# cbg-ethz/metMHN

Measured on AMD Instinct MI355X. Metric: full-cohort log-lik+grad evals/sec at n=20 events; kronvec HBM GB/s, higher is better.
Workload: dtype f64

## Files before the change

### include/metmhn_amd.h

```cpp
#ifndef METMHN_AMD_H
#define METMHN_AMD_H

#include <stddef.h>
#include <stdint.h>

#ifdef __cplusplus
extern "C" {
#endif

typedef struct mmhn_engine* mmhn_handle;

enum { MMHN_F64 = 0, MMHN_F32 = 1 };

int mmhn_create(int device_id, int n_mut, int dtype, mmhn_handle* out);
void mmhn_destroy(mmhn_handle h);
const char* mmhn_last_error(void);
int mmhn_set_workspace_limit(mmhn_handle h, size_t bytes);

int mmhn_set_cohort(mmhn_handle h, const int8_t* dat, int64_t n_pat, int n_cols);
int mmhn_score(mmhn_handle h, const double* log_theta, const double* log_d_p, const double* log_d_m,
               double perc_met, double* score);
int mmhn_score_and_grad(mmhn_handle h, const double* log_theta, const double* log_d_p,
                        const double* log_d_m, double perc_met, double* score, double* d_theta,
                        double* d_dp, double* d_dm);
// ... 83 lines not shown
                         double* pos_mt, int32_t* status);

int mmhn_order_samples(mmhn_handle h, const double* log_theta, const double* obs1, const double* obs2, const int8_t* dat,
                       int64_t n_pat, int n_cols, int64_t first, int64_t n_samples, uint64_t seed, double* log_evidence,
                       int8_t* orders, double* log_prob, int32_t* status);

enum { MMHN_K_OTHER_SOLVE = 0,
       MMHN_K_PSOLVE_FWD = 1,
       MMHN_K_PSOLVE_ADJ = 2,
       MMHN_K_PCLASS = 3,
       MMHN_K_CSOLVE_FWD = 4,
       MMHN_K_CSOLVE_ADJ = 5,
       MMHN_K_COUNT = 6 };
typedef struct {
  double ms;
  int64_t launches;
  double alg_bytes;
} mmhn_kernel_counter;
typedef struct {
  mmhn_kernel_counter kernel[MMHN_K_COUNT];
  double eval_ms;
  int64_t evals;
  int32_t comm_ranks;
  int32_t comm_rank;
} mmhn_counters;
#define MMHN_ABI_VERSION 8
int mmhn_abi_version(void);
int mmhn_bench_kronvec(mmhn_handle h, const double* log_theta, const int8_t* state, int64_t batch,
                       int iters, int transpose, int jacobi, double* ms_per_launch, int64_t* tiles);
int mmhn_bench_stream(mmhn_handle h, size_t bytes, int iters, int kind, double* gbps);
int mmhn_get_counters(mmhn_handle h, mmhn_counters* out);
int mmhn_reset_counters(mmhn_handle h);
int mmhn_debug_lane_moves(mmhn_handle h, int transposed, int* out);

#ifdef __cplusplus
}
#endif
#endif
```

### metmhn_amd/_lib.py

```python
from __future__ import annotations

import ctypes as C
import os
import subprocess

_HERE = os.path.dirname(os.path.abspath(__file__))
_ROOT = os.path.dirname(_HERE)
import glob
_SRC = [os.path.join(_HERE, "csrc", "engine.hip")] + sorted(glob.glob(os.path.join(_HERE, "csrc", "*.h")))
_HDR = os.path.join(_ROOT, "include", "metmhn_amd.h")
LIB_PATH = os.environ.get("MMHN_LIB", os.path.join(_HERE, "libmetmhn_amd.so"))

f64p = C.POINTER(C.c_double)
i8p = C.POINTER(C.c_int8)
i64p = C.POINTER(C.c_int64)
i32p = C.POINTER(C.c_int32)


KERNEL_CLASSES = ("other_solve", "psolve_fwd", "psolve_adj", "pclass", "csolve_fwd", "csolve_adj")


class KernelCounter(C.Structure):
    _fields_ = [("ms", C.c_double), ("launches", C.c_int64), ("alg_bytes", C.c_double)]

# ... 14 lines not shown
    "mmhn_cohort_sums_end": [C.c_void_p, f64p],
    "mmhn_cohort_wsums_begin": [C.c_void_p, f64p, f64p, f64p, C.c_int, C.c_double],
    "mmhn_cohort_wsums_end": [C.c_void_p, f64p],
    "mmhn_set_reduce_flag": [C.c_void_p, C.c_double],
    "mmhn_get_reduce_flag": [C.c_void_p, f64p],
    "mmhn_patient_grads": [C.c_void_p, f64p, f64p, f64p, f64p, f64p, f64p, f64p],
    "mmhn_kronvec": [C.c_void_p, f64p, i8p, f64p, f64p, C.c_int, C.c_int],
    "mmhn_kronvec_batched": [C.c_void_p, f64p, i8p, C.c_int64, f64p, f64p, C.c_int, C.c_int],
    "mmhn_jacobi_step_batched": [C.c_void_p, f64p, f64p, f64p, i8p, C.c_int64, f64p, f64p, f64p, C.c_int],
    "mmhn_kron_diag": [C.c_void_p, f64p, i8p, f64p],
    "mmhn_diag_scal": [C.c_void_p, f64p, i8p, f64p, f64p, C.c_int],
    "mmhn_obs_states": [C.c_void_p, i8p, C.c_int, i64p, i64p],
    "mmhn_resolvent": [C.c_void_p, f64p, f64p, f64p, i8p, f64p, f64p, C.c_int],
    "mmhn_x_partial_Q_y": [C.c_void_p, f64p, i8p, f64p, f64p, f64p],
    "mmhn_x_partial_D_y": [C.c_void_p, f64p, f64p, i8p, f64p, f64p, f64p, f64p],
    "mmhn_partial_diag_scal": [C.c_void_p, f64p, i8p, f64p, C.c_int, C.c_int, f64p],
    "mmhn_v_kronvec": [C.c_void_p, f64p, i8p, f64p, f64p, C.c_int, C.c_int],
    "mmhn_v_resolvent": [C.c_void_p, f64p, i8p, f64p, f64p, f64p, C.c_int],
    "mmhn_v_x_partial_Q_y": [C.c_void_p, f64p, i8p, f64p, f64p, f64p, f64p],
    "mmhn_v_kron_diag": [C.c_void_p, f64p, i8p, f64p, f64p],
    "mmhn_v_scal_d_pt": [C.c_void_p, f64p, f64p, i8p, f64p, f64p, f64p],
    "mmhn_v_d_scal_d_pt": [C.c_void_p, f64p, f64p, i8p, f64p, C.c_int, f64p, f64p],
    "mmhn_v_x_partial_D_y": [C.c_void_p, f64p, f64p, i8p, f64p, f64p, f64p, f64p],
    "mmhn_comm_unique_id": [C.c_void_p],
    "mmhn_comm_init": [C.c_void_p, C.c_void_p, C.c_int, C.c_int],
    "mmhn_comm_destroy": [C.c_void_p],
    "mmhn_bench_stream": [C.c_void_p, C.c_size_t, C.c_int, C.c_int, f64p],
    "mmhn_bench_kronvec": [C.c_void_p, f64p, i8p, C.c_int64, C.c_int, C.c_int, C.c_int, f64p, i64p],
    "mmhn_simulate": [C.c_void_p, f64p, f64p, f64p, C.c_int64, C.c_uint64, i8p, i8p],
    "mmhn_simulate_summary": [C.c_void_p, f64p, f64p, f64p, C.c_int64, C.c_int64, C.c_uint64, i64p],
    "mmhn_get_counters": [C.c_void_p, C.POINTER(Counters)],
    "mmhn_reset_counters": [C.c_void_p],
    "mmhn_debug_lane_moves": [C.c_void_p, C.c_int, C.POINTER(C.c_int)],
    "mmhn_likeliest_orders": [C.c_void_p, f64p, f64p, f64p, i8p, C.c_int64, C.c_int, C.c_int, i8p, f64p, i32p],
    "mmhn_order_posteriors": [C.c_void_p, f64p, f64p, f64p, i8p, C.c_int64, C.c_int, f64p, f64p, f64p, i32p],
    "mmhn_order_precedences": [C.c_void_p, f64p, f64p, f64p, i8p, C.c_int64, C.c_int, f64p, f64p, i32p],
    "mmhn_order_positions": [C.c_void_p, f64p, f64p, f64p, i8p, C.c_int64, C.c_int, f64p, f64p, f64p, i32p],
    "mmhn_order_samples": [C.c_void_p, f64p, f64p, f64p, i8p, C.c_int64, C.c_int, C.c_int64, C.c_int64, C.c_uint64, f64p, i8p,
                           f64p, i32p],
}
OTHER_SYMBOLS = ("mmhn_destroy", "mmhn_last_error", "mmhn_abi_version")
ABI_VERSION = 8


def needs_build() -> bool:
    if not os.path.exists(LIB_PATH):
        return True
    t = os.path.getmtime(LIB_PATH)
    return any(os.path.exists(s) and os.path.getmtime(s) > t for s in _SRC + [_HDR])


def build(force: bool = False, verbose: bool = False) -> str:
    if not force and not needs_build():
        return LIB_PATH
    hipcc = os.environ.get("HIPCC", "/opt/rocm/bin/hipcc")
    cmd = [hipcc, "-O3", "-std=c++17", "--offload-arch=gfx950", "-shared", "-fPIC", "-Wno-comment",
           "-o", LIB_PATH, _SRC[0]]
    if verbose:
        print(" ".join(cmd))
    res = subprocess.run(cmd, capture_output=True, text=True)
    if res.returncode != 0:
        raise RuntimeError("hipcc failed:\n" + res.stderr)
    return LIB_PATH


_lib = None
# ... 39 lines not shown
```

### metmhn_amd/csrc/engine.hip

```cpp
#include <algorithm>
#include <chrono>
#include <cmath>
#include <cstdio>
#include <cstdlib>
#include <cstring>
#include <string>
#include <vector>

#include "../../include/metmhn_amd.h"
#include "host.h"
#include "comm.h"
#include "plan.h"
#include "sampler.h"

namespace mmhn {

static thread_local std::string g_err;

struct CListDev {
  DevArr<CItem> items;
  DevArr<int> deps;
};
struct StagedDev {
  DevArr<int> pats, paired, probs;
// ... 87 lines not shown
  DevArr<T> piM, qM;
  DevArr<T> zarena;
  struct View { T* p = nullptr; } GJ, DJ, Abuf;
  int pi_owner = -1, qJ_owner = -1;
  DevArr<double> lp, out, sums, abi_sums, redbuf;
  DevArr<JLink<T>> links;
  double* h_abi = nullptr;
  double* h_abi_dev = nullptr;
  hipStream_t side[3] = {};
  hipEvent_t ev_fork[3] = {}, ev_join[3] = {};
  bool small_forked[2] = {false, false}, fork_recorded[2] = {false, false};
  DevArr<CoopCtl> coop_ctl;
  DevArr<unsigned> coop_flags[2];
  unsigned coop_epoch = 0;
  int coop_slot = 0;
  int cur_lane = 0;
  unsigned* h_abort = nullptr;
  unsigned* h_abort_dev = nullptr;
  bool coop_used = false;
  bool coop_alone = false;
  bool sums_pending = false;
  std::chrono::steady_clock::time_point sums_t0, sums_issued;
  int sums_len = 0;
  int pack_mode = 0;
  double pack_a = 0, pack_b = 0;
  double* pack_dst = nullptr;
  bool packed_in_eval = false;
  double reduce_flag = 0.0, reduce_flag_sum = 0.0;
  bool flag_pending = false;
  ncclComm_t comm = nullptr;
  int comm_rank = 0, comm_size = 1;
  bool time_kernels = true;
  mmhn_counters cnt{};
  std::vector<std::pair<hipEvent_t, hipEvent_t>> ev_pool;
  size_t ev_used = 0;
  std::vector<double> ev_bytes;
  std::vector<int> ev_slot;

  static long long zarena_elems(long long nJ, long long asize, int N) { return up4(3 * nJ * N * N) + up4(3 * nJ * N) + up4(asize); }
  static long long zclear_elems(const Batch& b, int N) { return zarena_elems((long long)b.dJ.size(), b.aclr, N); }

  Engine(int dev_id, int n_mut) : n(n_mut), N(n_mut + 1) {
    device = dev_id;
    cnt.comm_rank = -1;
    REQUIRE(n_mut >= 1 && n_mut < MAXN, "n_mut must be in [1, 31]");
    DevGuard guard(device);
    HIPCHECK(hipStreamCreateWithFlags(&stream, hipStreamNonBlocking));
    d_par.alloc(NPSET);
    HIPCHECK(hipHostMalloc(reinterpret_cast<void**>(&h_par), NPSET * sizeof(Params<T>), hipHostMallocDefault));
    HIPCHECK(hipHostGetDevicePointer(&h_par_dev, h_par, 0));
    static_assert(sizeof(Params<T>) % sizeof(uint4) == 0, "parameter block: whole 16-byte words");
    sums.alloc(2 * stride());
    size_t free_b = 0, total_b = 0;
    HIPCHECK(hipMemGetInfo(&free_b, &total_b));
    cfg.plan.ws_limit = (size_t)(0.7 * (double)free_b);
    hipDeviceProp_t prop;
    HIPCHECK(hipGetDeviceProperties(&prop, device));
    cfg.plan.n_cu = std::max(1, prop.multiProcessorCount);
    {
      std::vector<uint16_t> perm((size_t)(TB + 1) << TB, 0);
      std::vector<int> lvl((size_t)(TB + 1) * (TB + 2), 0);
      for (int t = 0; t <= TB; ++t) {
        int pos = 0;
        for (int l = 0; l <= t; ++l) {
          lvl[(size_t)t * (TB + 2) + l] = pos;
          for (uint32_t x = 0; x < (1u << t); ++x)
            if (popc(x) == l) perm[((size_t)t << TB) + pos++] = (uint16_t)x;
        }
        lvl[(size_t)t * (TB + 2) + t + 1] = pos;
      }
      d_perm.alloc(perm.size());
      d_lvl.alloc(lvl.size());
      HIPCHECK(hipMemcpy(d_perm.p, perm.data(), perm.size() * sizeof(uint16_t), hipMemcpyHostToDevice));
      HIPCHECK(hipMemcpy(d_lvl.p, lvl.data(), lvl.size() * sizeof(int), hipMemcpyHostToDevice));
    }
    raise_lds(wsolve_lds<T>(), &k_wsolve<T, false>, &k_wsolve<T, true>, &k_wsolve<T, false, WCfg<T>::NXT>, &k_wsolve<T, true, WCfg<T>::NXT>);
    raise_lds(wclass_lds<T>(), &k_wclass<T>);
    raise_lds(160 * 1024, &k_spatient2<T>, &k_spatient<T, 1024, 1>);
    raise_lds(150 * 1024,
              &k_csolve<T, false, false>, &k_csolve<T, true, false>, &k_csolve<T, false, true>, &k_csolve<T, true, true>,
              &k_csolve<T, false, false, 4>, &k_csolve<T, true, false, 4>,
              &k_psolve2<T, false, true>, &k_psolve2<T, true, true>, &k_psolve2<T, false, false>, &k_psolve2<T, true, false>,
              &k_tsolve<T, false, false>, &k_tsolve<T, true, false>, &k_tsolve<T, false, true>, &k_tsolve<T, true, true>,
              &k_kv<T, false, 1, false>, &k_kv<T, true, 1, false>, &k_kv<T, false, 1, true>, &k_kv<T, true, 1, true>,
              &k_sweep<T, false>, &k_sweep<T, true>, &k_diag<T>, &k_diag<T, 1024>,
              &k_prep<T, false>, &k_prep<T, true>, &k_prep<T, false, 1024>, &k_grad_rows<T, 1>, &k_grad_rows<T>,
              &k_pclass<T, false>, &k_pclass<T, true>, &k_class_marg<T>);
    coop_ctl.alloc(1);
    HIPCHECK(hipMemset(coop_ctl.p, 0, sizeof(CoopCtl)));
    HIPCHECK(hipHostMalloc(reinterpret_cast<void**>(&h_abort), 64, hipHostMallocDefault));
    HIPCHECK(hipHostGetDevicePointer(reinterpret_cast<void**>(&h_abort_dev), h_abort, 0));
    *h_abort = 0u;
    for (int i = 0; i < 3; ++i) {
      HIPCHECK(hipStreamCreateWithFlags(&side[i], hipStreamNonBlocking));
      HIPCHECK(hipEventCreateWithFlags(&ev_fork[i], hipEventDisableTiming));
      HIPCHECK(hipEventCreateWithFlags(&ev_join[i], hipEventDisableTiming));
    }
  }
  ~Engine() override {
    comm_destroy();
    for (auto& e : ev_pool) { (void)hipEventDestroy(e.first); (void)hipEventDestroy(e.second); }
    for (int i = 0; i < 3; ++i) {
      if (ev_join[i]) (void)hipEventDestroy(ev_join[i]);
      if (ev_fork[i]) (void)hipEventDestroy(ev_fork[i]);
      if (side[i]) (void)hipStreamDestroy(side[i]);
    }
    if (h_par) (void)hipHostFree(h_par);
    if (h_abi) (void)hipHostFree(h_abi);
    if (h_abort) (void)hipHostFree(h_abort);
    if (stream) (void)hipStreamDestroy(stream);
    stream = nullptr;
  }
  int stride() const { return 1 + N * N + 2 * N; }

  void build_params(const double* lt, const double* ldp, const double* ldm, bool upload = true) {
    REQUIRE(!sums_pending, "an evaluation begun with mmhn_cohort_sums_begin has not been collected (its parameter upload may still be in flight)");
    std::vector<double> eth((size_t)N * N), enp(N, 1.0), enm(N, 1.0);
    for (int e = 0; e < N * N; ++e) eth[e] = std::exp(lt[e]);
    if (ldp) for (int j = 0; j < N; ++j) enp[j] = std::exp(-ldp[j]);
// ... 67 lines not shown
#undef KV_ARGS
    HIPCHECK(hipGetLastError());
  }
  void collect_events() {
    for (size_t i = 0; i < ev_used; ++i) {
      float ms = 0;
      HIPCHECK(hipEventElapsedTime(&ms, ev_pool[i].first, ev_pool[i].second));
      mmhn_kernel_counter& c = cnt.kernel[ev_slot[i]];
      c.ms += ms;
      c.launches += 1;
      c.alg_bytes += ev_bytes[i];
    }
    ev_used = 0;
    ev_bytes.clear();
    ev_slot.clear();
  }

  void launch_diag(const Desc* descs, const int2* map, int ntiles, const T* p, T* outp, const T* dvec, int what,
                   int pbit = -1) {
    if (ntiles == 0) return;
    const size_t lds = DESC_PAD + ((size_t)4 * N * 64 + 256) * sizeof(T);
    if (ntiles >= 256)
      hipLaunchKernelGGL((k_diag<T, 1024>), dim3(ntiles), dim3(1024), lds, stream, descs, map, d_par.p, p, outp, dvec, what, N, pbit);
    else
      hipLaunchKernelGGL((k_diag<T>), dim3(ntiles), dim3(BLOCK), lds, stream, descs, map, d_par.p, p, outp, dvec,
                         what, N, pbit);
    HIPCHECK(hipGetLastError());
  }
  void launch_grad_rows(const Desc* descs, int nprob, int maxk, const T* A, const T* p, const T* q, T* G, int kind,
                        const DevArr<int2>& chunks, T* dj = nullptr, long long gstride = 0) {
    if (nprob == 0 || chunks.n == 0) return;
    (void)maxk;
    const int rows = N + (dj ? 1 : 0);
    if (chunks.n >= 1024) {
      const size_t lds1 = ((size_t)192 + 32) * sizeof(T);
      hipLaunchKernelGGL((k_grad_rows<T, 1>), dim3((unsigned)chunks.n, rows), dim3(64), lds1, stream,
                         descs, d_par.p, A, p, q, G, kind, dj, chunks.p, nprob, gstride);
      HIPCHECK(hipGetLastError());
      return;
    }
    const size_t lds = ((size_t)WAVES * 192 + WAVES * 32) * sizeof(T);
    hipLaunchKernelGGL((k_grad_rows<T>), dim3((unsigned)chunks.n, (rows + WAVES - 1) / WAVES), dim3(BLOCK), lds, stream,
                       descs, d_par.p, A, p, q, G, kind, dj, chunks.p, nprob, gstride);
    HIPCHECK(hipGetLastError());
  }
  void zero(T* p, long long count) {
    if (count > 0) HIPCHECK(hipMemsetAsync(p, 0, (size_t)count * sizeof(T), stream));
  }
  void poison_fill(T* p, long long count) {
    if (cfg.poison && count > 0) HIPCHECK(hipMemsetAsync(p, 0xFF, (size_t)count * sizeof(T), stream));
  }
  template <typename F>
  void timed(int slot, double alg_bytes, F&& launch) {
    if (!time_kernels) {
      launch();
      HIPCHECK(hipGetLastError());
      return;
    }
    if (ev_used == ev_pool.size()) {
      hipEvent_t a, b;
      HIPCHECK(hipEventCreate(&a));
      HIPCHECK(hipEventCreate(&b));
      ev_pool.push_back({a, b});
    }
    hipEvent_t e0 = ev_pool[ev_used].first, e1 = ev_pool[ev_used].second;
    ++ev_used;
    ev_bytes.push_back(alg_bytes);
    ev_slot.push_back(slot);
    HIPCHECK(hipEventRecord(e0, stream));
    launch();
    HIPCHECK(hipGetLastError());
    HIPCHECK(hipEventRecord(e1, stream));
  }

  size_t psolve2_lds(int maxk) const {
// ... 387 lines not shown
        HIPCHECK(hipGetLastError());
        if (pack_mode && &b == &batches.back()) {
          hipLaunchKernelGGL(k_reduce_parts_pack, dim3((st + BLOCK - 1) / BLOCK), dim3(BLOCK), 0, stream, redbuf.p, st, nelem, nchunk,
                             sums.p, pack_mode, N, pack_a, pack_b, pack_dst);
          packed_in_eval = true;
        } else {
          hipLaunchKernelGGL(k_reduce_parts, dim3(cols.x, 2), dim3(BLOCK), 0, stream, redbuf.p, st, nelem, nchunk, sums.p);
        }
        HIPCHECK(hipGetLastError());
      }
      if (host_out) {
        std::vector<double> tmp((size_t)npat * st);
        HIPCHECK(hipMemcpyAsync(tmp.data(), out.p, tmp.size() * sizeof(double), hipMemcpyDeviceToHost, stream));
        HIPCHECK(hipStreamSynchronize(stream));
        check_abort();
        for (int i = 0; i < npat; ++i)
          std::memcpy(host_out + (size_t)b.pats[i].row * st, tmp.data() + (size_t)i * st, st * sizeof(double));
      }
    }
    time_kernels = true;
    if (host_sums) {
      std::vector<double> hs(2 * st);
      HIPCHECK(hipMemcpyAsync(hs.data(), sums.p, hs.size() * sizeof(double), hipMemcpyDeviceToHost, stream));
      HIPCHECK(hipStreamSynchronize(stream));
      check_abort();
      std::memcpy(host_sums, hs.data(), hs.size() * sizeof(double));
      finish_eval(t0);
    }
  }
  void reset_counters() {
    const int r = cnt.comm_ranks, k = cnt.comm_rank;
    cnt = mmhn_counters{};
    cnt.comm_ranks = r; cnt.comm_rank = k;
  }
  void finish_eval(std::chrono::steady_clock::time_point t0) {
    collect_events();
    cnt.eval_ms += std::chrono::duration<double, std::milli>(std::chrono::steady_clock::now() - t0).count();
    cnt.evals += 1;
  }

  void cohort_sums_begin(const double* lt, const double* ldp, const double* ldm, bool grad, const double* w_combined = nullptr) {
    REQUIRE(!sums_pending, "mmhn_cohort_sums_begin: the previous evaluation has not been collected");
    sums_t0 = std::chrono::steady_clock::now();
    const int full = 4 + 2 * N * N + 3 * N;
    const int total = w_combined ? stride() : full;
    abi_sums.alloc(full);
    if (!h_abi) {
      HIPCHECK(hipHostMalloc(reinterpret_cast<void**>(&h_abi), (size_t)full * sizeof(double), hipHostMallocDefault));
      HIPCHECK(hipHostGetDevicePointer(reinterpret_cast<void**>(&h_abi_dev), h_abi, 0));
    }
    double* packed = (cfg.zero_copy && !comm) ? h_abi_dev : abi_sums.p;
    pack_mode = w_combined ? 2 : 1;
    pack_a = w_combined ? *w_combined : (double)n_em; pack_b = w_combined ? reduce_flag : (double)n_pat; pack_dst = packed;
    packed_in_eval = false;
    struct Unset { int& m; ~Unset() { m = 0; } } unset{pack_mode};
    evaluate(lt, ldp, ldm, grad, nullptr, nullptr);
    if (!packed_in_eval) {
      if (w_combined) hipLaunchKernelGGL(k_pack_wsums, dim3(2), dim3(256), 0, stream, sums.p, N, *w_combined, packed, reduce_flag);
      else hipLaunchKernelGGL(k_pack_sums, dim3(2), dim3(256), 0, stream, sums.p, N, n_em, (double)n_pat, packed);
      HIPCHECK(hipGetLastError());
    }
    const int moved = total + (w_combined ? 1 : 0);
    if (comm) RCCLCHECK(rccl().AllReduce(abi_sums.p, abi_sums.p, (size_t)moved, ncclFloat64, ncclSum, comm, stream));
    if (packed == abi_sums.p) HIPCHECK(hipMemcpyAsync(h_abi, abi_sums.p, moved * sizeof(double), hipMemcpyDeviceToHost, stream));
    flag_pending = w_combined != nullptr;
    reduce_flag = 0.0;
// ... 603 lines not shown
int mmhn_debug_stamps(mmhn_handle h, double* out16, int reset) {
  API_BEGIN
  GUARD(h);
  unsigned long long v[16];
  HIPCHECK(hipDeviceSynchronize());
  HIPCHECK(hipMemcpyFromSymbol(v, HIP_SYMBOL(g_stamps), sizeof(v)));
  for (int i = 0; i < 16; ++i) out16[i] = (double)v[i];
  if (reset) { std::memset(v, 0, sizeof(v)); HIPCHECK(hipMemcpyToSymbol(HIP_SYMBOL(g_stamps), v, sizeof(v))); }
  API_END
}
#endif
int mmhn_get_counters(mmhn_handle h, mmhn_counters* out) {
  API_BEGIN
  GUARD(h);
  REQUIRE(h && h->impl && out, "null pointer");
  if (h->dtype == MMHN_F64) *out = static_cast<Engine<double>*>(h->impl)->cnt;
  else *out = static_cast<Engine<float>*>(h->impl)->cnt;
  API_END
}
int mmhn_debug_lane_moves(mmhn_handle h, int transposed, int* out) {
  API_BEGIN
  GUARD(h);
  REQUIRE(out, "null pointer");
  DevArr<int> d;
  d.alloc(6 * 64);
  if (transposed) hipLaunchKernelGGL((k_lane_moves<true>), dim3(1), dim3(64), 0, h->impl->stream, d.p);
  else hipLaunchKernelGGL((k_lane_moves<false>), dim3(1), dim3(64), 0, h->impl->stream, d.p);
  HIPCHECK(hipGetLastError());
  HIPCHECK(hipMemcpyAsync(out, d.p, 6 * 64 * sizeof(int), hipMemcpyDeviceToHost, h->impl->stream));
  HIPCHECK(hipStreamSynchronize(h->impl->stream));
  API_END
}

int mmhn_abi_version(void) { return MMHN_ABI_VERSION; }

int mmhn_reset_counters(mmhn_handle h) {
  API_BEGIN
  GUARD(h);
  DISPATCH(h, reset_counters());
  API_END
}

}
```

### metmhn_amd/csrc/gradrows.h

```cpp
#pragma once
#include "common.h"

namespace mmhn {

enum { GK_P = 0, GK_M = 1, GK_E = 2, GK_S = 3 };

template <typename T>
__device__ __forceinline__ T wave_sum(T v) {
  for (int o = 32; o > 0; o >>= 1) v += __shfl_xor(v, o);
  return v;
}

template <int CTRL, int ROWMASK>
__device__ __forceinline__ double dpp_add(double v) {
  const int lo = __builtin_amdgcn_update_dpp(0, __double2loint(v), CTRL, ROWMASK, 0xF, false);
  const int hi = __builtin_amdgcn_update_dpp(0, __double2hiint(v), CTRL, ROWMASK, 0xF, false);
  return v + __hiloint2double(hi, lo);
}
template <int CTRL, int ROWMASK>
__device__ __forceinline__ float dpp_add(float v) {
  return v + __int_as_float(__builtin_amdgcn_update_dpp(0, __float_as_int(v), CTRL, ROWMASK, 0xF, false));
}
__device__ __forceinline__ double lane63(double v) {
  return __hiloint2double(__builtin_amdgcn_readlane(__double2hiint(v), 63), __builtin_amdgcn_readlane(__double2loint(v), 63));
// ... 11 lines not shown
}
template <int S, typename T>
__device__ __forceinline__ T dpp_stage(T v) {
  if constexpr (S == 0) return dpp_add<0xB1, 0xF>(v);
  else if constexpr (S == 1) return dpp_add<0x4E, 0xF>(v);
  else if constexpr (S == 2) return dpp_add<0x141, 0xF>(v);
  else if constexpr (S == 3) return dpp_add<0x140, 0xF>(v);
  else if constexpr (S == 4) return dpp_add<0x142, 0xA>(v);
  else return dpp_add<0x143, 0xC>(v);
}
template <int S, typename T>
__device__ __forceinline__ T dpp_stages_from(T v) {
  if constexpr (S < 6) return dpp_stages_from<S + 1>(dpp_stage<S>(v));
  else return v;
}
template <typename T>
__device__ __forceinline__ void wave_bit_sums(T v, int lane, int nb, T& total, T (&M)[6]) {
  const T p0 = v;
  const T p1 = dpp_stage<0>(p0), p2 = dpp_stage<1>(p1), p3 = dpp_stage<2>(p2), p4 = dpp_stage<3>(p3), p5 = dpp_stage<4>(p4);
  total = lane63(dpp_stage<5>(p5));
  if (nb > 0) M[0] = lane63(dpp_stages_from<0>((lane & 1) ? p0 : T(0)));
  if (nb > 1) M[1] = lane63(dpp_stages_from<1>((lane & 2) ? p1 : T(0)));
  if (nb > 2) M[2] = lane63(dpp_stages_from<2>((lane & 4) ? p2 : T(0)));
  if (nb > 3) M[3] = lane63(dpp_stages_from<3>((lane & 8) ? p3 : T(0)));
  if (nb > 4) M[4] = lane63(dpp_stages_from<4>((lane & 16) ? p4 : T(0)));
  if (nb > 5) M[5] = lane63(dpp_stages_from<5>((lane & 32) ? p5 : T(0)));
}

__device__ __forceinline__ double lane_bcast(double v, int src) {
  return __hiloint2double(__builtin_amdgcn_readlane(__double2hiint(v), src), __builtin_amdgcn_readlane(__double2loint(v), src));
}
__device__ __forceinline__ float lane_bcast(float v, int src) { return __int_as_float(__builtin_amdgcn_readlane(__float_as_int(v), src)); }

constexpr int GR_CHUNK = 11;

template <typename T, int GW = WAVES>
__global__ __launch_bounds__(GW * 64) void k_grad_rows(const Desc* __restrict__ descs,
                                                     const Params<T>* __restrict__ par,
                                                     const T* __restrict__ A,
                                                     const T* __restrict__ p,
                                                     const T* __restrict__ q, T* G, int kind_arg,
                                                     T* DJ, const int2* __restrict__ chunks,
                                                     int nprob, long long gstride) {
  extern __shared__ __align__(16) unsigned char smem[];
  T* Tlo = reinterpret_cast<T*>(smem);
  T* rowbuf = Tlo + GW * 192;
  __shared__ int lev[32];
  const int prob = chunks[blockIdx.x].x;
  const int kind = kind_arg < 0 ? chunks[blockIdx.x].y >> 24 : kind_arg;
  const int chunk = chunks[blockIdx.x].y & 0xffffff;
  if (kind_arg < 0) G += (long long)kind * gstride;
  const Desc& d = descs[prob];
  const int N = d.N, n = N - 1;
  const int tid = threadIdx.x, w = tid >> 6, lane = tid & 63;
  const int i = blockIdx.y * GW + w;
  const Params<T>& P = par[d.pset];

  uint32_t cm;
  if (kind == GK_P) cm = d.maskP; else if (kind == GK_M) cm = d.maskM;
  else if (kind == GK_E) cm = d.pairP; else cm = (1u << d.k) - 1u;
  const int kc = __popc(cm);
  if (tid < kc) {
    uint32_t m = cm;
    for (int q = 0; q < tid; ++q) m &= m - 1;
    lev[tid] = d.ev[__ffs(m) - 1];
  }
  __syncthreads();
  const bool drow = i == N;
  if (i > N || (drow && (kind == GK_S || DJ == nullptr))) return;
  T* row = drow ? DJ + ((long long)kind * nprob + prob) * N : G + ((long long)prob * N + i) * N;
  T* rb = rowbuf + w * 32;
  if (lane < 32) rb[lane] = 0;
  const T* fvec = drow ? (kind == GK_M ? P.dm : P.dp) : P.th[i < N ? i : 0];

  bool rowvalid = true;
  T base = drow ? (kind == GK_P ? -P.dp[n] : kind == GK_M ? -P.dm[n] : T(-1)) : (kind == GK_M ? P.baseM[i] : P.baseP[i]);
  if ((kind == GK_P || kind == GK_M) && ((!drow && i >= n) || d.seedbit < 0)) rowvalid = false;
  if (kind == GK_E && d.mode != JOINT) rowvalid = false;
  int slot = -1;
  if (drow) slot = -1;
  else if (kind == GK_E && i == n) slot = kc;
  else for (int l = 0; l < kc; ++l) if (lev[l] == i) slot = l;

  if (rowvalid) {
    const int klo = kc < 6 ? kc : 6;
    const int kin = kc < GR_CHUNK ? kc : GR_CHUNK;
    const int nhi = kin - klo;
    const T fl = lane < kc ? fvec[lev[lane < kc ? lane : 0]] : T(1);
#pragma unroll
    for (int part = 0; part < 3; ++part) {
      T v = 1;
#pragma unroll
      for (int l = 0; l < 6; ++l) {
        const int ll = part * 6 + l;
        const T f = lane_bcast(fl, ll);
        if (ll < kc && ((lane >> l) & 1)) v *= f;
      }
      Tlo[w * 192 + part * 64 + lane] = v;
    }
    constexpr int NHI = GR_CHUNK - 6;
    T ha[NHI];
#pragma unroll
    for (int l = 0; l < NHI; ++l) ha[l] = 0;
    const T* Ab = nullptr;
    if (kind != GK_S) {
      long long o = d.aoff;
      if (kind != GK_P) o += class_block_size(__popc(d.maskP));
      if (kind == GK_E) o += class_block_size(__popc(d.maskM));
      Ab = A + o;
    }
    const long long nS = 1ll << kc;
    const long long Sbeg = (long long)chunk << GR_CHUNK;
    const long long Send = nS < Sbeg + (1ll << GR_CHUNK) ? nS : Sbeg + (1ll << GR_CHUNK);
    T tot = 0;
    constexpr int GU = 4;
    for (long long S00 = Sbeg; S00 < Send; S00 += 64 * GU) {
      T a0[GU], a1[GU];
      bool live[GU];
#pragma unroll
      for (int u = 0; u < GU; ++u) {
        const long long S = S00 + 64 * u + lane;
        const uint32_t s = (uint32_t)S;
        const bool blocked = slot >= 0 && slot < kc && ((s >> slot) & 1u);
        live[u] = S < nS && !blocked;
        a0[u] = 0; a1[u] = 0;
        if (live[u]) {
          if (kind == GK_S) {
            const T pv = p[d.off + s];
            a0[u] = -pv * q[d.off + s];
            if (slot >= 0) a1[u] = pv * q[d.off + (s | (1u << slot))];
          } else {
            a0[u] = Ab[S];
            if (slot >= 0) a1[u] = Ab[((long long)(slot + 1) << kc) + S];
          }
        }
      }
#pragma unroll
      for (int u = 0; u < GU; ++u) {
        const long long S0 = S00 + 64 * u;
        if (S0 >= nS) break;
        const uint32_t s = (uint32_t)(S0 + lane);
        T urate = base;
        urate *= Tlo[w * 192 + 64 + ((S0 >> 6) & 63)] * Tlo[w * 192 + 128 + ((S0 >> 12) & 63)];
        for (int l = 18; l < kc; ++l) if ((S0 >> l) & 1) urate *= fvec[lev[l]];
        const T f = live[u] ? urate * Tlo[w * 192 + (s & 63u)] * (a0[u] + a1[u]) : T(0);
        tot += f;
#pragma unroll
        for (int l = 0; l < NHI; ++l) if (l < nhi && ((S0 >> (6 + l)) & 1)) ha[l] += f;
      }
    }
    const T total = wave_sum(tot);
    if (lane == 0) {
      if (drow) { if (kind != GK_E) rb[n] = total; }
      else { rb[i] = total; if (kind == GK_M) rb[n] = total; }
    }
    for (int l = 0; l < klo; ++l) {
      const T m = wave_sum(((lane >> l) & 1) ? tot : T(0));
      if (lane == 0 && lev[l] != i) rb[lev[l]] = m;
    }
#pragma unroll
    for (int l = 0; l < NHI; ++l) {
      if (l < nhi) {
        const T m = wave_sum(ha[l]);
        if (lane == 0 && lev[6 + l] != i) rb[lev[6 + l]] = m;
      }
    }
    if (lane == 0)
      for (int l = kin; l < kc; ++l)
        if (((Sbeg >> l) & 1) && lev[l] != i) rb[lev[l]] = total;
  }
  if (lane < N && rb[lane] != T(0)) atomicAdd(&row[lane], rb[lane]);
}

template <typename T>
__global__ __launch_bounds__(BLOCK) void k_bit_marg(const Desc* __restrict__ descs,
                                                    const int2* __restrict__ map,
                                                    const Params<T>* __restrict__ par,
                                                    const T* __restrict__ p,
                                                    const T* __restrict__ q, T* out) {
  __shared__ T part[WAVES][2][16];
  const Desc& d = descs[map[blockIdx.x].x];
  const uint32_t H = (uint32_t)map[blockIdx.x].y;
  const int k = d.k, n = d.N - 1;
  const int t = k < TB ? k : TB;
  const uint32_t nelem = 1u << t;
  const Params<T>& P = par[d.pset];
  const bool joint = d.mode == JOINT;
  const int tid = threadIdx.x, w = tid >> 6, lane = tid & 63;
  constexpr int NJ = (1 << TB) / BLOCK;
  T tot[2] = {0, 0};
  T mj[2][4] = {{0, 0, 0, 0}, {0, 0, 0, 0}};
#pragma unroll
  for (int j = 0; j < NJ; ++j) {
    const uint32_t xl = (uint32_t)j * BLOCK + tid;
    if (xl < nelem) {
      const uint32_t x = (H << t) | xl;
      T a = 1, b = 1;
      for (int bb = 0; bb < k; ++bb)
        if ((x >> bb) & 1u) {
          if (joint ? d.cls[bb] == CP : bb != d.seedbit) a *= P.dp[d.ev[bb]];
          if (joint ? d.cls[bb] == CM : bb != d.seedbit) b *= P.dm[d.ev[bb]];
        }
      const bool sbit = d.seedbit >= 0 && ((x >> d.seedbit) & 1u);
      T wA, wB;
// ... 40 lines not shown
```

### metmhn_amd/engine.py

```python
from __future__ import annotations

import ctypes as C

import numpy as np

from . import _lib
from ._lib import f64p, i8p, i64p

F64, F32 = 0, 1
_DEFAULT = {"device": None}


def set_default_device(device: int | None):
    _DEFAULT["device"] = None if device is None else int(device)


def default_device() -> int:
    if _DEFAULT["device"] is not None:
        return _DEFAULT["device"]
    import os
    return int(os.environ.get("LOCAL_RANK", "0"))


def unique_id() -> bytes:
# ... 378 lines not shown
                                               orders.ctypes.data_as(i8p), log_prob.ctypes.data_as(f64p),
                                               status.ctypes.data_as(_lib.i32p)))
        return le, orders, log_prob, status

    def bench_kronvec(self, log_theta, state, batch, iters, transpose=False, jacobi=False, tiles=False):
        lt, ltp = _f(log_theta); st, sp = _s(state)
        ms = C.c_double()
        tl = (C.c_int64 * 2)()
        _lib.check(self.lib.mmhn_bench_kronvec(self.h, ltp, sp, int(batch), int(iters), int(transpose), int(jacobi),
                                               C.byref(ms), tl))
        return (ms.value, int(tl[0]), int(tl[1])) if tiles else ms.value

    def bench_stream(self, nbytes=1 << 30, iters=10, kind="copy"):
        out = C.c_double()
        _lib.check(self.lib.mmhn_bench_stream(self.h, int(nbytes), int(iters), 0 if kind == "copy" else 1, C.byref(out)))
        return out.value

    def counters(self):
        c = _lib.Counters()
        _lib.check(self.lib.mmhn_get_counters(self.h, C.byref(c)))
        out = {"eval_ms": c.eval_ms, "evals": c.evals, "comm_ranks": int(c.comm_ranks), "comm_rank": int(c.comm_rank)}
        for i, name in enumerate(_lib.KERNEL_CLASSES):
            k = c.kernel[i]
            out[name] = {"ms": k.ms, "launches": k.launches, "alg_bytes": k.alg_bytes}
        return out

    def reset_counters(self):
        _lib.check(self.lib.mmhn_reset_counters(self.h))

    def debug_lane_moves(self, transposed=False):
        out = (C.c_int * (6 * 64))()
        _lib.check(self.lib.mmhn_debug_lane_moves(self.h, int(bool(transposed)), out))
        return np.array(out[:], dtype=np.int64).reshape(6, 64)
```

Baseline: 21.95.

## Restructure grad-rows kernel into single-wave row loops with register-resident data

Rewrites the gradient-row kernel so each 64-thread wave loops over several gradient rows with a grid-stride over rows, sized from the CU count, instead of one wave per row. For small classes the state vector is kept in registers and reused across rows. The next row's data is prefetched while the current row is reduced. Shared-memory tables are replaced by lane broadcasts, and direct stores replace atomics when a single chunk covers the class. It also adds a debug counter API for launch shapes. The cost is more register pressure and more complex control flow.

```diff
diff --git a/include/metmhn_amd.h b/include/metmhn_amd.h
--- a/include/metmhn_amd.h
+++ b/include/metmhn_amd.h
@@ -139,6 +139,7 @@
 int mmhn_get_counters(mmhn_handle h, mmhn_counters* out);
 int mmhn_reset_counters(mmhn_handle h);
 int mmhn_debug_lane_moves(mmhn_handle h, int transposed, int* out);
+int mmhn_debug_grad_rows(mmhn_handle h, int64_t* out);
 
 #ifdef __cplusplus
 }
diff --git a/metmhn_amd/_lib.py b/metmhn_amd/_lib.py
--- a/metmhn_amd/_lib.py
+++ b/metmhn_amd/_lib.py
@@ -70,6 +70,7 @@
     "mmhn_get_counters": [C.c_void_p, C.POINTER(Counters)],
     "mmhn_reset_counters": [C.c_void_p],
     "mmhn_debug_lane_moves": [C.c_void_p, C.c_int, C.POINTER(C.c_int)],
+    "mmhn_debug_grad_rows": [C.c_void_p, i64p],
     "mmhn_likeliest_orders": [C.c_void_p, f64p, f64p, f64p, i8p, C.c_int64, C.c_int, C.c_int, i8p, f64p, i32p],
     "mmhn_order_posteriors": [C.c_void_p, f64p, f64p, f64p, i8p, C.c_int64, C.c_int, f64p, f64p, f64p, i32p],
     "mmhn_order_precedences": [C.c_void_p, f64p, f64p, f64p, i8p, C.c_int64, C.c_int, f64p, f64p, i32p],
diff --git a/metmhn_amd/csrc/engine.hip b/metmhn_amd/csrc/engine.hip
--- a/metmhn_amd/csrc/engine.hip
+++ b/metmhn_amd/csrc/engine.hip
@@ -143,6 +143,7 @@
   int comm_rank = 0, comm_size = 1;
   bool time_kernels = true;
   mmhn_counters cnt{};
+  long long gr_stat[8] = {0, 0, 0, 0, 0, 0, 0, 0};
   std::vector<std::pair<hipEvent_t, hipEvent_t>> ev_pool;
   size_t ev_used = 0;
   std::vector<double> ev_bytes;
@@ -195,7 +196,7 @@
               &k_tsolve<T, false, false>, &k_tsolve<T, true, false>, &k_tsolve<T, false, true>, &k_tsolve<T, true, true>,
               &k_kv<T, false, 1, false>, &k_kv<T, true, 1, false>, &k_kv<T, false, 1, true>, &k_kv<T, true, 1, true>,
               &k_sweep<T, false>, &k_sweep<T, true>, &k_diag<T>, &k_diag<T, 1024>,
-              &k_prep<T, false>, &k_prep<T, true>, &k_prep<T, false, 1024>, &k_grad_rows<T, 1>, &k_grad_rows<T>,
+              &k_prep<T, false>, &k_prep<T, true>, &k_prep<T, false, 1024>,
               &k_pclass<T, false>, &k_pclass<T, true>, &k_class_marg<T>);
     coop_ctl.alloc(1);
     HIPCHECK(hipMemset(coop_ctl.p, 0, sizeof(CoopCtl)));
@@ -329,15 +330,11 @@
     if (nprob == 0 || chunks.n == 0) return;
     (void)maxk;
     const int rows = N + (dj ? 1 : 0);
-    if (chunks.n >= 1024) {
-      const size_t lds1 = ((size_t)192 + 32) * sizeof(T);
-      hipLaunchKernelGGL((k_grad_rows<T, 1>), dim3((unsigned)chunks.n, rows), dim3(64), lds1, stream,
-                         descs, d_par.p, A, p, q, G, kind, dj, chunks.p, nprob, gstride);
-      HIPCHECK(hipGetLastError());
-      return;
-    }
-    const size_t lds = ((size_t)WAVES * 192 + WAVES * 32) * sizeof(T);
-    hipLaunchKernelGGL((k_grad_rows<T>), dim3((unsigned)chunks.n, (rows + WAVES - 1) / WAVES), dim3(BLOCK), lds, stream,
+    const long long want = (long long)cfg.plan.n_cu * 24;
+    const int Y = (int)std::max<long long>(1, std::min<long long>(rows, want / (long long)chunks.n));
+    long long* st = gr_stat + (kind < 0 ? 0 : 4);
+    st[Y == 1 ? 0 : 1] += 1; st[2] = Y; st[3] = (long long)chunks.n;
+    hipLaunchKernelGGL((k_grad_rows<T>), dim3((unsigned)chunks.n, Y), dim3(64), 0, stream,
                        descs, d_par.p, A, p, q, G, kind, dj, chunks.p, nprob, gstride);
     HIPCHECK(hipGetLastError());
   }
@@ -791,6 +788,7 @@
     const int r = cnt.comm_ranks, k = cnt.comm_rank;
     cnt = mmhn_counters{};
     cnt.comm_ranks = r; cnt.comm_rank = k;
+    for (long long& v : gr_stat) v = 0;
   }
   void finish_eval(std::chrono::steady_clock::time_point t0) {
     collect_events();
@@ -1460,6 +1458,15 @@
   API_END
 }
 
+int mmhn_debug_grad_rows(mmhn_handle h, int64_t* out) {
+  API_BEGIN
+  GUARD(h);
+  REQUIRE(h && h->impl && out, "null pointer");
+  const long long* st = h->dtype == MMHN_F64 ? static_cast<Engine<double>*>(h->impl)->gr_stat : static_cast<Engine<float>*>(h->impl)->gr_stat;
+  for (int i = 0; i < 8; ++i) out[i] = st[i];
+  API_END
+}
+
 int mmhn_abi_version(void) { return MMHN_ABI_VERSION; }
 
 int mmhn_reset_counters(mmhn_handle h) {
diff --git a/metmhn_amd/csrc/gradrows.h b/metmhn_amd/csrc/gradrows.h
--- a/metmhn_amd/csrc/gradrows.h
+++ b/metmhn_amd/csrc/gradrows.h
@@ -67,144 +67,210 @@
 }
 __device__ __forceinline__ float lane_bcast(float v, int src) { return __int_as_float(__builtin_amdgcn_readlane(__float_as_int(v), src)); }
 
+__device__ __forceinline__ int lane_bcast(int v, int src) { return __builtin_amdgcn_readlane(v, src); }
+
 constexpr int GR_CHUNK = 11;
-
-template <typename T, int GW = WAVES>
-__global__ __launch_bounds__(GW * 64) void k_grad_rows(const Desc* __restrict__ descs,
-                                                     const Params<T>* __restrict__ par,
-                                                     const T* __restrict__ A,
-                                                     const T* __restrict__ p,
-                                                     const T* __restrict__ q, T* G, int kind_arg,
-                                                     T* DJ, const int2* __restrict__ chunks,
-                                                     int nprob, long long gstride) {
-  extern __shared__ __align__(16) unsigned char smem[];
-  T* Tlo = reinterpret_cast<T*>(smem);
-  T* rowbuf = Tlo + GW * 192;
-  __shared__ int lev[32];
+constexpr int GR_RES = 9;
+
+template <typename T, bool RES>
+__device__ __forceinline__ void grad_rows_item(const Desc& d, const Params<T>& P, const T* __restrict__ Ab,
+                                               const T* __restrict__ p, const T* __restrict__ q, T* Gp, T* djrow,
+                                               const int kind, const int kc, const int levl, const int chunk,
+                                               const int i0, const int Y, const int rows) {
+  const int lane = threadIdx.x, N = d.N, n = N - 1;
+  const bool pm = kind == GK_P || kind == GK_M;
+  const int klo = kc < 6 ? kc : 6;
+  const int kin = kc < GR_CHUNK ? kc : GR_CHUNK;
+  const int nhi = kin - klo;
+  constexpr int NHI = GR_CHUNK - 6;
+  const uint32_t nS = 1u << kc, Sbeg = (uint32_t)chunk << GR_CHUNK;
+  const uint32_t Send = nS < Sbeg + (1u << GR_CHUNK) ? nS : Sbeg + (1u << GR_CHUNK);
+  constexpr int GU = RES ? (1 << GR_RES) / 64 : 4;
+  const int ng = (int)((Send - Sbeg + 63u) >> 6);
+  const long long off = d.off;
+
+  T r0[GU], r1[GU], rp[GU];
+#pragma unroll
+  for (int u = 0; u < GU; ++u) { r0[u] = 0; r1[u] = 0; rp[u] = 0; }
+  auto load0 = [&](int u, uint32_t S00, bool all) {
+    const uint32_t S = S00 + 64u * u + (uint32_t)lane;
+    if (all) {
+      if (kind == GK_S) { rp[u] = p[off + S]; r0[u] = q[off + S]; }
+      else r0[u] = Ab[S];
+    }
+  };
+  auto load1 = [&](int u, uint32_t S00, int slot) {
+    const uint32_t S = S00 + 64u * u + (uint32_t)lane;
+    const bool blocked = slot >= 0 && slot < kc && ((S >> slot) & 1u);
+    const bool live = S < nS && !blocked;
+    if (!RES) load0(u, S00, live);
+    if (live && slot >= 0) r1[u] = kind == GK_S ? q[off + (S | (1u << slot))] : Ab[((long long)(slot + 1) << kc) + S];
+  };
+  auto slot_of = [&](int i) -> int {
+    if (i == N) return -1;
+    if (kind == GK_E && i == n) return kc;
+    const unsigned long long b = __ballot(lane < kc && levl == i);
+    return b ? __ffsll(b) - 1 : -1;
+  };
+  auto row_load = [&](int i, T& fl, T& base) {
+    const bool drow = i == N;
+    const T* fvec = drow ? (kind == GK_M ? P.dm : P.dp) : P.th[i];
+    fl = lane < kc ? fvec[levl] : T(1);
+    base = drow ? (kind == GK_P ? -P.dp[n] : kind == GK_M ? -P.dm[n] : T(-1)) : (kind == GK_M ? P.baseM[i] : P.baseP[i]);
+  };
+  auto next_row = [&](int i) -> int { i += Y; if (pm && i == n) i += Y; return i; };
+
+  int i = i0;
+  if (pm && i == n) i += Y;
+  if (i >= rows) return;
+  if (RES) {
+#pragma unroll
+    for (int u = 0; u < GU; ++u) if (u < ng) load0(u, 0u, 64u * u + (uint32_t)lane < nS);
+  }
+  T fl, base;
+  row_load(i, fl, base);
+  int slot = slot_of(i);
+#pragma unroll
+  for (int u = 0; u < GU; ++u) if (u < ng) load1(u, Sbeg, slot);
+  if (RES && kind == GK_S) {
+#pragma unroll
+    for (int u = 0; u < GU; ++u) r0[u] = -rp[u] * r0[u];
+  }
+
+  for (;;) {
+    const bool drow = i == N;
+    T v0 = 1, v1 = 1, v2 = 1;
+#pragma unroll
+    for (int l = 0; l < 6; ++l) {
+      const T f = lane_bcast(fl, l);
+      if (l < kc && ((lane >> l) & 1)) v0 *= f;
+    }
+    if (kc > 6) {
+#pragma unroll
+      for (int l = 0; l < 6; ++l) {
+        const T f = lane_bcast(fl, 6 + l);
+        if (6 + l < kc && ((lane >> l) & 1)) v1 *= f;
+      }
+    }
+    if (kc > 12) {
+#pragma unroll
+      for (int l = 0; l < 6; ++l) {
+        const T f = lane_bcast(fl, 12 + l);
+        if (12 + l < kc && ((lane >> l) & 1)) v2 *= f;
+      }
+    }
+    const T c2 = lane_bcast(v2, (int)((Sbeg >> 12) & 63u));
+    T tot = 0, ha[NHI];
+#pragma unroll
+    for (int l = 0; l < NHI; ++l) ha[l] = 0;
+    auto group = [&](uint32_t S0, T a0, T a1) {
+      const uint32_t S = S0 + (uint32_t)lane;
+      const bool blocked = slot >= 0 && slot < kc && ((S >> slot) & 1u);
+      T urate = base * (lane_bcast(v1, (int)((S0 >> 6) & 63u)) * c2);
+      for (int l = 18; l < kc; ++l) if ((S0 >> l) & 1u) urate *= lane_bcast(fl, l);
+      const T f = (S < nS && !blocked) ? urate * v0 * (a0 + a1) : T(0);
+      tot += f;
+#pragma unroll
+      for (int l = 0; l < NHI; ++l) if (l < nhi && ((S0 >> (6 + l)) & 1u)) ha[l] += f;
+    };
+    auto cooked0 = [&](int u) -> T { return (!RES && kind == GK_S) ? -rp[u] * r0[u] : r0[u]; };
+    auto cooked1 = [&](int u) -> T { return slot < 0 ? T(0) : kind == GK_S ? rp[u] * r1[u] : r1[u]; };
+#pragma unroll
+    for (int u = 0; u < GU; ++u) if (u < ng) group(Sbeg + 64u * u, cooked0(u), cooked1(u));
+    if (!RES) {
+      for (uint32_t S00 = Sbeg + 64u * GU; S00 < Send; S00 += 64u * GU) {
+#pragma unroll
+        for (int u = 0; u < GU; ++u) load1(u, S00, slot);
+#pragma unroll
+        for (int u = 0; u < GU; ++u) group(S00 + 64u * u, cooked0(u), cooked1(u));
+      }
+    }
+    const int inx = next_row(i);
+    const bool more = inx < rows;
+    T fln = 1, basen = 0;
+    int slotn = -1;
+    if (more) {
+      row_load(inx, fln, basen);
+      slotn = slot_of(inx);
+#pragma unroll
+      for (int u = 0; u < GU; ++u) if (u < ng) load1(u, Sbeg, slotn);
+    }
+    T total, ML[6];
+    wave_bit_sums(tot, lane, klo, total, ML);
+    T mine = 0;
+    if (drow) { if (kind != GK_E && lane == n) mine = total; }
+    else if (lane == i || (kind == GK_M && lane == n)) mine = total;
+#pragma unroll
+    for (int l = 0; l < 6; ++l) {
+      if (l < klo) {
+        const int e = lane_bcast(levl, l);
+        if (lane == e && e != i) mine = ML[l];
+      }
+    }
+#pragma unroll
+    for (int h = 0; h < NHI; ++h) {
+      if (h < nhi) {
+        const T m = wave_sum_dpp(ha[h]);
+        const int e = lane_bcast(levl, 6 + h);
+        if (lane == e && e != i) mine = m;
+      }
+    }
+    for (int l = kin; l < kc; ++l) {
+      if ((Sbeg >> l) & 1u) {
+        const int e = lane_bcast(levl, l);
+        if (lane == e && e != i) mine = total;
+      }
+    }
+    T* row = drow ? djrow : Gp + (long long)i * N;
+    if (lane < N) {
+      if (kc <= GR_CHUNK) row[lane] = mine;
+      else if (mine != T(0)) atomicAdd(&row[lane], mine);
+    }
+    if (!more) break;
+    i = inx; fl = fln; base = basen; slot = slotn;
+  }
+}
+
+template <typename T>
+__global__ __launch_bounds__(64) void k_grad_rows(const Desc* __restrict__ descs,
+                                                  const Params<T>* __restrict__ par,
+                                                  const T* __restrict__ A,
+                                                  const T* __restrict__ p,
+                                                  const T* __restrict__ q, T* G, int kind_arg,
+                                                  T* DJ, const int2* __restrict__ chunks,
+                                                  int nprob, long long gstride) {
   const int prob = chunks[blockIdx.x].x;
   const int kind = kind_arg < 0 ? chunks[blockIdx.x].y >> 24 : kind_arg;
   const int chunk = chunks[blockIdx.x].y & 0xffffff;
   if (kind_arg < 0) G += (long long)kind * gstride;
   const Desc& d = descs[prob];
-  const int N = d.N, n = N - 1;
-  const int tid = threadIdx.x, w = tid >> 6, lane = tid & 63;
-  const int i = blockIdx.y * GW + w;
+  const int N = d.N, lane = threadIdx.x;
   const Params<T>& P = par[d.pset];
 
   uint32_t cm;
   if (kind == GK_P) cm = d.maskP; else if (kind == GK_M) cm = d.maskM;
   else if (kind == GK_E) cm = d.pairP; else cm = (1u << d.k) - 1u;
   const int kc = __popc(cm);
-  if (tid < kc) {
+  if ((kind == GK_P || kind == GK_M) && d.seedbit < 0) return;
+  if (kind == GK_E && d.mode != JOINT) return;
+  const int rows = N + ((kind != GK_S && DJ != nullptr) ? 1 : 0);
+  int levl = 0;
+  if (lane < kc) {
     uint32_t m = cm;
-    for (int q = 0; q < tid; ++q) m &= m - 1;
-    lev[tid] = d.ev[__ffs(m) - 1];
-  }
-  __syncthreads();
-  const bool drow = i == N;
-  if (i > N || (drow && (kind == GK_S || DJ == nullptr))) return;
-  T* row = drow ? DJ + ((long long)kind * nprob + prob) * N : G + ((long long)prob * N + i) * N;
-  T* rb = rowbuf + w * 32;
-  if (lane < 32) rb[lane] = 0;
-  const T* fvec = drow ? (kind == GK_M ? P.dm : P.dp) : P.th[i < N ? i : 0];
-
-  bool rowvalid = true;
-  T base = drow ? (kind == GK_P ? -P.dp[n] : kind == GK_M ? -P.dm[n] : T(-1)) : (kind == GK_M ? P.baseM[i] : P.baseP[i]);
-  if ((kind == GK_P || kind == GK_M) && ((!drow && i >= n) || d.seedbit < 0)) rowvalid = false;
-  if (kind == GK_E && d.mode != JOINT) rowvalid = false;
-  int slot = -1;
-  if (drow) slot = -1;
-  else if (kind == GK_E && i == n) slot = kc;
-  else for (int l = 0; l < kc; ++l) if (lev[l] == i) slot = l;
-
-  if (rowvalid) {
-    const int klo = kc < 6 ? kc : 6;
-    const int kin = kc < GR_CHUNK ? kc : GR_CHUNK;
-    const int nhi = kin - klo;
-    const T fl = lane < kc ? fvec[lev[lane < kc ? lane : 0]] : T(1);
-#pragma unroll
-    for (int part = 0; part < 3; ++part) {
-      T v = 1;
-#pragma unroll
-      for (int l = 0; l < 6; ++l) {
-        const int ll = part * 6 + l;
-        const T f = lane_bcast(fl, ll);
-        if (ll < kc && ((lane >> l) & 1)) v *= f;
-      }
-      Tlo[w * 192 + part * 64 + lane] = v;
-    }
-    constexpr int NHI = GR_CHUNK - 6;
-    T ha[NHI];
-#pragma unroll
-    for (int l = 0; l < NHI; ++l) ha[l] = 0;
-    const T* Ab = nullptr;
-    if (kind != GK_S) {
-      long long o = d.aoff;
-      if (kind != GK_P) o += class_block_size(__popc(d.maskP));
-      if (kind == GK_E) o += class_block_size(__popc(d.maskM));
-      Ab = A + o;
-    }
-    const long long nS = 1ll << kc;
-    const long long Sbeg = (long long)chunk << GR_CHUNK;
-    const long long Send = nS < Sbeg + (1ll << GR_CHUNK) ? nS : Sbeg + (1ll << GR_CHUNK);
-    T tot = 0;
-    constexpr int GU = 4;
-    for (long long S00 = Sbeg; S00 < Send; S00 += 64 * GU) {
-      T a0[GU], a1[GU];
-      bool live[GU];
-#pragma unroll
-      for (int u = 0; u < GU; ++u) {
-        const long long S = S00 + 64 * u + lane;
-        const uint32_t s = (uint32_t)S;
-        const bool blocked = slot >= 0 && slot < kc && ((s >> slot) & 1u);
-        live[u] = S < nS && !blocked;
-        a0[u] = 0; a1[u] = 0;
-        if (live[u]) {
-          if (kind == GK_S) {
-            const T pv = p[d.off + s];
-            a0[u] = -pv * q[d.off + s];
-            if (slot >= 0) a1[u] = pv * q[d.off + (s | (1u << slot))];
-          } else {
-            a0[u] = Ab[S];
-            if (slot >= 0) a1[u] = Ab[((long long)(slot + 1) << kc) + S];
-          }
-        }
-      }
-#pragma unroll
-      for (int u = 0; u < GU; ++u) {
-        const long long S0 = S00 + 64 * u;
-        if (S0 >= nS) break;
-        const uint32_t s = (uint32_t)(S0 + lane);
-        T urate = base;
-        urate *= Tlo[w * 192 + 64 + ((S0 >> 6) & 63)] * Tlo[w * 192 + 128 + ((S0 >> 12) & 63)];
-        for (int l = 18; l < kc; ++l) if ((S0 >> l) & 1) urate *= fvec[lev[l]];
-        const T f = live[u] ? urate * Tlo[w * 192 + (s & 63u)] * (a0[u] + a1[u]) : T(0);
-        tot += f;
-#pragma unroll
-        for (int l = 0; l < NHI; ++l) if (l < nhi && ((S0 >> (6 + l)) & 1)) ha[l] += f;
-      }
-    }
-    const T total = wave_sum(tot);
-    if (lane == 0) {
-      if (drow) { if (kind != GK_E) rb[n] = total; }
-      else { rb[i] = total; if (kind == GK_M) rb[n] = total; }
-    }
-    for (int l = 0; l < klo; ++l) {
-      const T m = wave_sum(((lane >> l) & 1) ? tot : T(0));
-      if (lane == 0 && lev[l] != i) rb[lev[l]] = m;
-    }
-#pragma unroll
-    for (int l = 0; l < NHI; ++l) {
-      if (l < nhi) {
-        const T m = wave_sum(ha[l]);
-        if (lane == 0 && lev[6 + l] != i) rb[lev[6 + l]] = m;
-      }
-    }
-    if (lane == 0)
-      for (int l = kin; l < kc; ++l)
-        if (((Sbeg >> l) & 1) && lev[l] != i) rb[lev[l]] = total;
-  }
-  if (lane < N && rb[lane] != T(0)) atomicAdd(&row[lane], rb[lane]);
+    for (int b = 0; b < lane; ++b) m &= m - 1;
+    levl = d.ev[__ffs(m) - 1];
+  }
+  const T* Ab = nullptr;
+  if (kind != GK_S) {
+    long long o = d.aoff;
+    if (kind != GK_P) o += class_block_size(__popc(d.maskP));
+    if (kind == GK_E) o += class_block_size(__popc(d.maskM));
+    Ab = A + o;
+  }
+  T* Gp = G + (long long)prob * N * N;
+  T* djrow = DJ ? DJ + ((long long)kind * nprob + prob) * N : nullptr;
+  if (kc <= GR_RES) grad_rows_item<T, true>(d, P, Ab, p, q, Gp, djrow, kind, kc, levl, chunk, (int)blockIdx.y, (int)gridDim.y, rows);
+  else grad_rows_item<T, false>(d, P, Ab, p, q, Gp, djrow, kind, kc, levl, chunk, (int)blockIdx.y, (int)gridDim.y, rows);
 }
 
 template <typename T>
diff --git a/metmhn_amd/engine.py b/metmhn_amd/engine.py
--- a/metmhn_amd/engine.py
+++ b/metmhn_amd/engine.py
@@ -434,3 +434,10 @@
         out = (C.c_int * (6 * 64))()
         _lib.check(self.lib.mmhn_debug_lane_moves(self.h, int(bool(transposed)), out))
         return np.array(out[:], dtype=np.int64).reshape(6, 64)
+
+    def debug_grad_rows(self):
+        out = (C.c_int64 * 8)()
+        _lib.check(self.lib.mmhn_debug_grad_rows(self.h, out))
+        v = [int(x) for x in out]
+        return {name: {"launches_y1": v[o], "launches_ygt1": v[o + 1], "last_y": v[o + 2], "last_items": v[o + 3]}
+                for name, o in (("joint", 0), ("single", 4))}
```

Result: no change. 22.01 (median of 6 runs) (+0.3%).
